# smritip/real-time-audio-sync

Measured on AMD Instinct MI355X. Metric: aligned chroma frames/sec, batch=64 OTW c=500; path-index match vs CPU ref, higher is better.
Workload: dtype f64 arithmetic, f32 features in HBM

## Files before the change

real_time_audio_sync_amd/csrc/otw.hip:

```cpp
#include <hip/hip_runtime.h>
#include <math.h>
#include <stddef.h>
#include <stdint.h>
#include <stdlib.h>
#include <string.h>
#include <type_traits>

#include "common.h"
#include "cost.h"

namespace rts {

constexpr int kF = 12;
constexpr int kFetch = 8;

struct OtwArgs {
    const void *ref;
    const void *live;
    const int32_t *live_len;
    int32_t *state;
    int32_t *path;
    double *bands;
    long long live_stride;
    int N, c, max_run_count, variant, cost_kind, mode;
// ... 89 lines not shown
__device__ __forceinline__ double wave_shift_up(double v, double lane0) {
    const int lo = __builtin_amdgcn_update_dpp(__double2loint(lane0), __double2loint(v), 0x138, 0xf, 0xf, false);
    const int hi = __builtin_amdgcn_update_dpp(__double2hiint(lane0), __double2hiint(v), 0x138, 0xf, 0xf, false);
    return __hiloint2double(hi, lo);
}

__device__ __forceinline__ double wave_bcast(double v, int src_lane) {
    const int lo = __builtin_amdgcn_readlane(__double2loint(v), src_lane);
    const int hi = __builtin_amdgcn_readlane(__double2hiint(v), src_lane);
    return __hiloint2double(hi, lo);
}

__device__ __forceinline__ double rfl(double v) {
    const int lo = __builtin_amdgcn_readfirstlane(__double2loint(v));
    const int hi = __builtin_amdgcn_readfirstlane(__double2hiint(v));
    return __hiloint2double(hi, lo);
}

#define RTS_DPP_MIN_STEP(CTRL, ROWMASK)                                                                       \
    do {                                                                                                      \
        const int tlo = __builtin_amdgcn_update_dpp(__double2loint(x), __double2loint(x), CTRL, ROWMASK, 0xf, false); \
        const int thi = __builtin_amdgcn_update_dpp(__double2hiint(x), __double2hiint(x), CTRL, ROWMASK, 0xf, false); \
        x = vmin(x, __hiloint2double(thi, tlo));                                                              \
    } while (0)

__device__ __forceinline__ double wave_min(double x) {
    RTS_DPP_MIN_STEP(0x111, 0xf);
    RTS_DPP_MIN_STEP(0x112, 0xf);
    RTS_DPP_MIN_STEP(0x114, 0xf);
    RTS_DPP_MIN_STEP(0x118, 0xf);
    RTS_DPP_MIN_STEP(0x142, 0xa);
    RTS_DPP_MIN_STEP(0x143, 0xc);
    return wave_bcast(x, 63);
}

__device__ __forceinline__ unsigned lds_addr(const double *p) {
    return (unsigned)(uintptr_t)(__attribute__((address_space(3))) const double *)p;
}
template <int OFF>
__device__ __forceinline__ double lds_read_imm(unsigned addr) {
    double r;
    asm volatile("ds_read_b64 %0, %1 offset:%2" : "=v"(r) : "v"(addr), "n"(OFF));
    return r;
}
template <int OFF>
__device__ __forceinline__ void lds_write_imm(unsigned addr, double v) {
    asm volatile("ds_write_b64 %0, %1 offset:%2" ::"v"(addr), "v"(v), "n"(OFF) : "memory");
}
template <int L, int R, int M = 0>
__device__ __forceinline__ void chain_load(unsigned bA, unsigned bB, unsigned dA, unsigned dB, double (&prevb)[L + 1],
                                           double (&D)[L]) {
    if constexpr (M <= L) {
        constexpr int off = ((R + M) & (L - 1)) * 65 * 8;
        constexpr bool wrap = (R + M) >= L;
        prevb[M] = lds_read_imm<off>(wrap ? bB : bA);
        if constexpr (M > 0) D[M - 1] = lds_read_imm<off>(wrap ? dB : dA);
        chain_load<L, R, M + 1>(bA, bB, dA, dB, prevb, D);
    }
}
template <int L, int M = 0>
__device__ __forceinline__ void chain_wait(double (&prevb)[L + 1], double (&D)[L]) {
    if constexpr (M == 0) asm volatile("s_waitcnt lgkmcnt(0)" ::: "memory");
    if constexpr (M <= L) {
        asm volatile("" : "+v"(prevb[M]));
        if constexpr (M < L) asm volatile("" : "+v"(D[M]));
        chain_wait<L, M + 1>(prevb, D);
// ... 748 lines not shown
template <int W, bool ALT>
__device__ __forceinline__ void otw_spec_strip(const double *Dv, const double *band, double *shadow, int pos, int c,
                                               int lane, double sentinel, OtwSpecOut *out, long long *rounds_acc = nullptr,
                                               bool prev0_sentinel = false) {
    const int k1 = (pos - c + 1 > 0) ? pos - c + 1 : 0;
    double fm;
    int fi;
    const double d_last = Dv[swz<W>(pos)];
    const double d_next = Dv[swz<W>(pos + 1)];
    int alt_ok = 0;
    strip_chain<W, false, true, ALT, true>(Dv, band, shadow, k1, pos - k1, (k1 > 0) ? sentinel : (double)INFINITY, lane, k1,
                                           fm, fi, nullptr, nullptr, 0, rounds_acc, prev0_sentinel, sentinel, &alt_ok);
    out->pmin[lane] = fm;
    out->pidx[lane] = fi;
    if (lane == 0) {
        out->k1 = k1;
        out->d = d_last;
        out->d2 = d_next;
        out->flag = alt_ok;
    }
}

template <int W>
__device__ __forceinline__ void otw_spec_argmin(double lm, int ml, int k1, double &g_out, int &idx_out) {
    constexpr int L = W / 64;
    const double g = wave_min(lm);
    const unsigned long long mask = __ballot(lm == g);
    const bool some = (g < INFINITY) && (mask != 0);
    const int first = (int)__builtin_ctzll(mask | (1ull << 63));
    g_out = g;
    idx_out = some ? k1 + L * first + __builtin_amdgcn_readlane(ml, first) : 0x7fffffff;
}

__device__ __forceinline__ double otw_last_cell_from(double prev_raw, int pos, int k1, double side_v, double diag_v, double d,
                                                     double sentinel) {
    const double inf = INFINITY;
    const int n = pos - k1;
    const double prev = (n > 0) ? prev_raw : ((k1 > 0) ? sentinel : inf);
    const double diag = (pos > 0) ? diag_v + 2 * d : inf;
    return vmin(vmin(side_v + d, diag), prev + d);
}
template <int W>
__device__ __forceinline__ double otw_last_cell(const double *band, int pos, int k1, double side_v, double diag_v, double d,
                                                double sentinel) {
    const int n = pos - k1;
    return otw_last_cell_from(band[swz<W>(pos - (n > 0 ? 1 : 0))], pos, k1, side_v, diag_v, d, sentinel);
}

template <int W, typename RT>
__device__ __forceinline__ OtwSettled otw_settle_hit_both(double *R, double *C, const OtwSpecOut *exr, const OtwSpecOut *exc,
                                                          OtwCtl &k, const OtwEnv &e, int pt, int j0, double sentinel) {
    const int c = e.c, lane = e.lane;
    const int jn = j0 + 1, t0 = pt - 1;
    if (e.deferred_update && k.pend_dir != -2) {
        k.run_count = (k.pend_dir == k.prev) ? k.run_count + 1 : 1;
        if (k.pend_dir != RTS_DIR_BOTH) k.prev = k.pend_dir;
        k.pend_dir = -2;
    }
    const int k1r_ = (j0 - c + 1 > 0) ? j0 - c + 1 : 0, k1c_ = (pt - c + 1 > 0) ? pt - c + 1 : 0;
    const double pra_raw = R[swz<W>(j0 - (j0 - k1r_ > 0 ? 1 : 0))], prb_raw = C[swz<W>(t0 - (t0 - k1c_ > 0 ? 1 : 0))];
    const double d1_raw = exr->d, d2_raw = exc->d, d3_raw = exc->d2, rlm = exr->pmin[lane], clm = exc->pmin[lane];
    const int rml = exr->pidx[lane], cml = exc->pidx[lane], rk1 = exr->k1, ck1 = exc->k1;
    const double d1 = rfl(d1_raw), d2 = rfl(d2_raw), d3 = rfl(d3_raw);
    double rmin, cmin;
    int ridx, cidx;
    otw_spec_argmin<W>(rlm, rml, __builtin_amdgcn_readfirstlane(rk1), rmin, ridx);
// ... 102 lines not shown
    k.cA = cl;
    k.cells += n + 1;
    OtwSettled o;
    o.row_fresh = is_row;
    o.col_fresh = !is_row;
    o.rf_min = o.cf_min = smin;
    o.rf_idx = o.cf_idx = sidx;
    o.row_corner = o.col_corner = true;
    o.rc = o.cc = cl;
    o.stop = false;
    return o;
}

#ifdef RTS_OTW_FULL_BARRIER
#define RTS_STEP_BARRIER() __syncthreads()
#else
#define RTS_STEP_BARRIER() ::rts::lds_barrier()
#endif

template <int W, int NW, bool DENSE, typename RT, bool SPEC>
__global__ void __launch_bounds__(64 * NW) __attribute__((amdgpu_waves_per_eu(kThroughput<RT> ? 6 : 1)))
otw_advance_kernel(OtwArgs a) {
    static_assert(!SPEC || (NW >= 8 && !DENSE), "the pipelined kernel needs 8 waves and no dense mirror");
    constexpr int NT = 64 * NW;
    constexpr int HW0 = SPEC ? 3 : (NW >= 4) ? 2 : 0;
    constexpr int NHELP = 64 * (NW - HW0);
#if defined(RTS_OTW_STAMPS) && RTS_OTW_STAMPS == 1
    long long stamp_sum[16] = {0, 0, 0, 0, 0, 0, 0, 0, 0, 0, 0, 0, 0, 0, 0, 0};
    int stamp_base = 0;
    long long stamp_last = (long long)__builtin_amdgcn_s_memtime();
    __builtin_amdgcn_s_waitcnt(0xC07F);
#endif
#if defined(RTS_OTW_STAMPS) && RTS_OTW_STAMPS == 2
    long long lw_hit = 0, lb_hit = 0, lw_oth = 0, lb_oth = 0, ln_hit = 0, ln_oth = 0, l_last = 0;
    long long lo_work = 0, lo_t0 = 0;
    long long lo_rounds = 0;
#define RTS_ROUNDS_ACC (&lo_rounds)
#define RTS_LW_BEGIN() do { lo_t0 = (long long)__builtin_amdgcn_s_memtime(); __builtin_amdgcn_s_waitcnt(0xC07F); } while (0)
#define RTS_LW_END(hit) do { const long long t_ = (long long)__builtin_amdgcn_s_memtime(); __builtin_amdgcn_s_waitcnt(0xC07F); if (hit) lo_work += t_ - lo_t0; } while (0)
#else
#define RTS_ROUNDS_ACC nullptr
#define RTS_LW_BEGIN() do { } while (0)
#define RTS_LW_END(hit) do { } while (0)
#endif
    extern __shared__ __align__(16) unsigned char smem_raw[];
    OtwLds<W, RT> &S = *reinterpret_cast<OtwLds<W, RT> *>(smem_raw);
    using LdsT = OtwLds<W, RT>;
    constexpr bool kNoLiveRing = !kHasLiveRing<RT>;
    constexpr bool kRefRing = !SPEC && !kNoLiveRing;
    constexpr size_t kSpecOff = (offsetof(LdsT, refw) + 15) & ~(size_t)15;
    OtwSpecLds<W> &SP = *reinterpret_cast<OtwSpecLds<W> *>(smem_raw + kSpecOff);

    const int tid = threadIdx.x;
    const int lane = tid & 63;
    const int wave = __builtin_amdgcn_readfirstlane(tid >> 6);
    const double sentinel = (a.variant == RTS_VARIANT_OTW) ? 1e10 : (double)INFINITY;
    const double inf = INFINITY;
    OtwEnv e;
    e.b = blockIdx.x;
    e.lane = lane;
    e.c = a.c;
    e.euclid = a.cost_kind == RTS_COST_EUCLID;
    e.variant = a.variant;
    e.mode = a.mode;
    e.max_run_count = a.max_run_count;
    e.path_cap = a.path_cap;
    e.live_f64 = a.live_f64;
    e.ref_f64 = a.ref_f64;
    e.live_base = (long long)e.b * a.live_stride * kF;
    e.live = a.live;
    if (a.ref_first) {
        const int nb = a.ref_len[e.b];
        e.N = nb;
        e.live_cap = 2 * nb;
        e.ref = static_cast<const char *>(a.ref) + a.ref_first[e.b] * (long long)kF * (a.ref_f64 ? 8 : 4);
    } else {
// ... 145 lines not shown
            S.j = k.j;
        }
    }
    __syncthreads();
    int buf = 0;
    OtwPlan pl;
    pl.t = pl.j0 = 0;
    pl.flags = kPlanExit;
    if constexpr (SPEC) {
        otw_costs_prime<W, RT>(S, e, S.t, S.j, tid, NT);
        if (wave == 0) {
            k.cA = rfl(S.R[swz<W>(k.j)]);
            k.cU = (k.t > 0) ? rfl(S.C[swz<W>(k.t - 1)]) : inf;
            k.cL = (k.j > 0) ? rfl(S.R[swz<W>(k.j - 1)]) : inf;
            pl = otw_make_plan<W, RT>(S, k, e, true);
        }
    } else {
        otw_precompute<W, RT>(S, e, S.t, S.j, S.Dr[0], S.Dc[0], tid, NT);
        if (wave == 0) otw_make_plan<W, RT>(S, k, e);
    }
    __syncthreads();

    int sp = 0;
#ifdef RTS_OTW_PRIO_W0
    if constexpr (SPEC) {
        if (wave == 0) __builtin_amdgcn_s_setprio(RTS_OTW_PRIO_W0);
        if (wave == 1 || wave == 2) __builtin_amdgcn_s_setprio(RTS_OTW_PRIO_W12);
    }
#endif
    if constexpr (SPEC) {
        if (wave >= HW0) {
            for (;;) {
                const int pt = __builtin_amdgcn_readfirstlane(S.plan_t[sp]), j0 = __builtin_amdgcn_readfirstlane(S.plan_j0[sp]);
                const int pflags = otw_resolve_plan(__builtin_amdgcn_readfirstlane(S.plan_flags[sp]), pt, c, &SP.col[sp]);
                if (pflags & kPlanExit) break;
                const bool do_row = (pflags & kPlanRow) != 0, do_col = (pflags & kPlanCol) != 0;
                RTS_LW_BEGIN();
                if constexpr (!kNoLiveRing)
                    if (wave == HW0) otw_refill<W, RT>(S, k, e, pt + 3, 0, false);
                if (!(pflags & kPlanHit)) RTS_STEP_BARRIER();
                if (!(pflags & kPlanStop))
                    otw_costs_advance<W, RT>(S, e, pt, j0 + (do_col ? 1 : 0), do_row, do_col, tid - 64 * HW0, NHELP);
                RTS_LW_END(pflags & kPlanHit);
                RTS_STEP_BARRIER();
                sp ^= 1;
            }
        } else if (wave == 1) {
            for (;;) {
                const int pt = __builtin_amdgcn_readfirstlane(S.plan_t[sp]), j0 = __builtin_amdgcn_readfirstlane(S.plan_j0[sp]);
                const int pflags = otw_resolve_plan(__builtin_amdgcn_readfirstlane(S.plan_flags[sp]), pt, c, &SP.col[sp]);
                if (pflags & kPlanExit) break;
                const int jn = j0 + ((pflags & kPlanCol) ? 1 : 0);
                double *R = (pflags & kPlanRi) ? SP.ShR : S.R, *Rsh = (pflags & kPlanRi) ? S.R : SP.ShR;
                RTS_LW_BEGIN();
                if (!(pflags & kPlanHit)) {
                    if ((pflags & (kPlanRow | kPlanCol | kPlanStop)) == (kPlanRow | kPlanCol))
                        otw_col_strip<W, DENSE, RT>(S, (pflags & kPlanCi) ? SP.ShC : S.C, a, e, S.Dc[(j0 + 1) & 1], pt,
                                                    j0 + 1, true, sentinel);
                    RTS_STEP_BARRIER();
                }
                if ((pflags & (kPlanHit | kPlanRow | kPlanCol)) == (kPlanHit | kPlanRow | kPlanCol)) {
                    const double av = otw_last_cell<W>(R, j0, (j0 - c + 1 > 0) ? j0 - c + 1 : 0, Rsh[swz<W>(j0)],
                                                       Rsh[swz<W>(j0 > 0 ? j0 - 1 : 0)], SP.row[sp].d, sentinel);
                    if (lane == 0) R[swz<W>(j0)] = av;
                }
                if (!(pflags & kPlanStop) && pt + 1 < live_len && pt + 1 < e.live_cap)
                    otw_spec_strip<W, false>(S.Dr[(pt + 1) & 1], R, Rsh, jn, c, lane, sentinel, &SP.row[sp ^ 1], RTS_ROUNDS_ACC);
                RTS_LW_END(pflags & kPlanHit);
                RTS_STEP_BARRIER();
                sp ^= 1;
            }
        } else if (wave == 2) {
            for (;;) {
                const int pt = __builtin_amdgcn_readfirstlane(S.plan_t[sp]), j0 = __builtin_amdgcn_readfirstlane(S.plan_j0[sp]);
                const int pflags = otw_resolve_plan(__builtin_amdgcn_readfirstlane(S.plan_flags[sp]), pt, c, &SP.col[sp]);
                if (pflags & kPlanExit) break;
                const int jn = j0 + ((pflags & kPlanCol) ? 1 : 0);
                double *C = (pflags & kPlanCi) ? SP.ShC : S.C, *Csh = (pflags & kPlanCi) ? S.C : SP.ShC;
                RTS_LW_BEGIN();
                if (!(pflags & kPlanHit)) {
                    if constexpr (kThroughput<RT>) {
                        const bool stop2 = (pflags & kPlanStop) != 0;
                        if (pflags & kPlanRow) {
                            double rf_min = inf;
                            int rf_idx = 0x7fffffff;
                            otw_row_strip<W, DENSE, RT>((pflags & kPlanRi) ? SP.ShR : S.R, a, e, S.Dr[pt & 1], pt, j0, jn, sentinel,
                                                        rf_min, rf_idx);
                            if (lane == 0) {
                                S.rfresh_min = rf_min;
                                S.rfresh_idx = rf_idx;
                            }
                        } else if ((pflags & kPlanCol) && !stop2) {
                            otw_col_strip<W, DENSE, RT>(S, C, a, e, S.Dc[jn & 1], pt, jn, false, sentinel);
                        }
                    }
                    RTS_STEP_BARRIER();
                }
                bool drop = false;
                if ((pflags & (kPlanHit | kPlanRow | kPlanCol)) == (kPlanHit | kPlanRow | kPlanCol)) {
                    const int t0 = pt - 1;
                    const double bv = otw_last_cell<W>(C, t0, (pt - c + 1 > 0) ? pt - c + 1 : 0, Csh[swz<W>(t0)],
                                                       Csh[swz<W>(t0 > 0 ? t0 - 1 : 0)], SP.col[sp].d, sentinel);
                    if (lane == 0) C[swz<W>(t0)] = bv;
                    drop = pt >= c;
                }
                if (!(pflags & kPlanStop) && jn + 1 < N)
                    otw_spec_strip<W, true>(S.Dc[(jn + 1) & 1], C, Csh, pt, c, lane, sentinel, &SP.col[sp ^ 1], RTS_ROUNDS_ACC, drop);
                RTS_LW_END(pflags & kPlanHit);
                RTS_STEP_BARRIER();
                sp ^= 1;
            }
        } else {
#if defined(RTS_OTW_STAMPS) && RTS_OTW_STAMPS == 2
            l_last = (long long)__builtin_amdgcn_s_memtime();
            __builtin_amdgcn_s_waitcnt(0xC07F);
#define RTS_W0_STEP_END(hit)                                              \
    do {                                                                  \
        const long long t0_ = (long long)__builtin_amdgcn_s_memtime();    \
        __builtin_amdgcn_s_waitcnt(0xC07F);                               \
        RTS_STEP_BARRIER();                                               \
        const long long t1_ = (long long)__builtin_amdgcn_s_memtime();    \
        __builtin_amdgcn_s_waitcnt(0xC07F);                               \
        if (hit) {                                                        \
            lw_hit += t0_ - l_last;                                       \
            lb_hit += t1_ - t0_;                                          \
            ln_hit += 1;                                                  \
        } else {                                                          \
            lw_oth += t0_ - l_last;                                       \
            lb_oth += t1_ - t0_;                                          \
            ln_oth += 1;                                                  \
        }                                                                 \
        l_last = t1_;                                                     \
    } while (0)
#else
#define RTS_W0_STEP_END(hit) RTS_STEP_BARRIER()
#endif
            int2 *const path_row = reinterpret_cast<int2 *>(e.path) + (size_t)e.b * e.path_cap;
            const auto hit_steps = [&](auto v2_c, auto defer_c) __attribute__((always_inline)) {
                constexpr bool V2 = decltype(v2_c)::value, DEFER = decltype(defer_c)::value;
#define RTS_RFL_CTL(f) k.f = __builtin_amdgcn_readfirstlane(k.f)
                RTS_RFL_CTL(t), RTS_RFL_CTL(j), RTS_RFL_CTL(dir), RTS_RFL_CTL(prev), RTS_RFL_CTL(run_count);
                RTS_RFL_CTL(status), RTS_RFL_CTL(n_path), RTS_RFL_CTL(consumed), RTS_RFL_CTL(rows), RTS_RFL_CTL(cols);
                RTS_RFL_CTL(truncated), RTS_RFL_CTL(pend_dir), RTS_RFL_CTL(pending_col), RTS_RFL_CTL(last_x);
                RTS_RFL_CTL(last_y), RTS_RFL_CTL(spec_valid), RTS_RFL_CTL(ri), RTS_RFL_CTL(ci);
#undef RTS_RFL_CTL
                for (;;) {
                    const int pt = __builtin_amdgcn_readfirstlane(pl.t), j0 = __builtin_amdgcn_readfirstlane(pl.j0);
                    const int fl = __builtin_amdgcn_readfirstlane(pl.flags);
                    const int kind = fl & (kPlanHit | kPlanRow | kPlanCol | kPlanStop | kPlanExit | kPlanHitIf);
                    const bool is_row = kind == (kPlanHit | kPlanRow);
                    if (!is_row && kind != (kPlanHit | kPlanCol)) return;
                    const int jn = is_row ? j0 : j0 + 1;
                    const int keep_lo = is_row ? pt - c + 1 : jn - c + 1;
                    const int keep_idx = __builtin_amdgcn_readfirstlane(is_row ? k.cb_idx : k.rb_idx);
                    if (keep_idx < ((keep_lo > 0) ? keep_lo : 0)) return;
#if defined(RTS_OTW_STAMPS) && RTS_OTW_STAMPS == 1
                    stamp_base = 0;
                    stamp_sum[6] += 1;
#endif
                    RTS_STAMP(0);
                    RTS_STAMP(1);
                    double *R = (fl & kPlanRi) ? SP.ShR : S.R, *C = (fl & kPlanCi) ? SP.ShC : S.C;
                    const int pos = is_row ? j0 : pt;
                    const int k1 = (pos - c + 1 > 0) ? pos - c + 1 : 0;
                    const int n = pos - k1;
                    double *band = is_row ? R : C, *other = is_row ? C : R;
                    const OtwSpecOut *ex = is_row ? &SP.row[sp] : &SP.col[sp];
                    if constexpr (DEFER) {
                        if (k.pend_dir != -2) {
                            k.run_count = (k.pend_dir == k.prev) ? k.run_count + 1 : 1;
                            if (k.pend_dir != RTS_DIR_BOTH) k.prev = k.pend_dir;
                            k.pend_dir = -2;
                        }
                    }
                    const double prev_raw = band[swz<W>(pos - (n > 0 ? 1 : 0))];
                    const double d = ex->d, lm = ex->pmin[lane];
                    const int ml = ex->pidx[lane], sk1 = ex->k1;
                    double smin;
                    int sidx;
                    otw_spec_argmin<W>(lm, ml, __builtin_amdgcn_readfirstlane(sk1), smin, sidx);
                    const double prev = (n > 0) ? prev_raw : ((k1 > 0) ? sentinel : inf);
                    const double diag = (pos > 0) ? (is_row ? k.cL : k.cU) + 2 * d : inf;
                    const double cl = vmin(vmin(k.cA + d, diag), prev + d);
                    if (lane == 0) {
                        band[swz<W>(pos)] = cl;
                        other[swz<W>(is_row ? pt : jn)] = cl;
                    }
                    if (is_row) {
                        k.rows += 1;
                        k.consumed = pt + 1;
                        k.cU = k.cA;
                        k.cL = prev;
                    } else {
                        k.cols += 1;
                        k.cL = k.cA;
                        k.cU = prev;
                    }
                    k.cA = cl;
                    k.cells += n + 1;
                    RTS_STAMP(3);
                    double rmin = is_row ? smin : k.rb_min, cmin = is_row ? k.cb_min : smin;
                    int ridx = is_row ? sidx : k.rb_idx, cidx = is_row ? k.cb_idx : sidx;
                    const bool r_new = cl < rmin, c_new = cl < cmin;
                    rmin = r_new ? cl : rmin;
                    ridx = r_new ? jn : ridx;
                    cmin = c_new ? cl : cmin;
                    cidx = c_new ? pt : cidx;
                    k.rb_min = rmin;
                    k.rb_idx = ridx;
                    k.cb_min = cmin;
                    k.cb_idx = cidx;
                    const bool rlt = rmin < cmin;
                    const int x = rlt ? pt : cidx, y = rlt ? ridx : jn;
                    bool append = true;
                    if constexpr (V2) {
                        const int xs = __builtin_amdgcn_readfirstlane(x), ys = __builtin_amdgcn_readfirstlane(y);
                        append = (k.n_path == 0) || (xs > k.last_x && ys >= k.last_y);
                        if (append) {
                            k.last_x = xs;
                            k.last_y = ys;
                        }
                    }
                    if (append) {
                        if (k.n_path < e.path_cap) {
                            if (lane == 0) path_row[k.n_path] = make_int2(x, y);
                        } else {
                            k.truncated = 1;
                        }
                        k.n_path += 1;
                    }
                    int nd = __builtin_amdgcn_readfirstlane((x < pt) ? RTS_DIR_COLUMN : (y < jn) ? RTS_DIR_ROW : RTS_DIR_BOTH);
                    if (pt < c)
                        nd = RTS_DIR_BOTH;
                    else if (k.run_count >= e.max_run_count)
                        nd = (k.prev == RTS_DIR_ROW) ? RTS_DIR_COLUMN : RTS_DIR_ROW;
                    if constexpr (DEFER) {
                        k.pend_dir = nd;
                    } else {
                        k.run_count = (nd == k.prev) ? k.run_count + 1 : 1;
                        if (nd != RTS_DIR_BOTH) k.prev = nd;
                    }
                    k.dir = nd;
                    k.pending_col = (nd == RTS_DIR_COLUMN);
                    k.t = pt;
                    k.j = jn;
                    RTS_STAMP(4);
                    k.spec_valid = 1;
                    pl = otw_make_plan<W, RT>(S, k, e, true, sp ^ 1);
                    RTS_STAMP(5);
                    RTS_W0_STEP_END(true);
                    sp ^= 1;
                }
            };
            for (;;) {
                if constexpr (W == 512 && !kThroughput<RT>) {
                    if (e.variant == RTS_VARIANT_LIVENOTE_V2) {
                        if (e.deferred_update)
                            hit_steps(std::true_type{}, std::true_type{});
                        else
                            hit_steps(std::true_type{}, std::false_type{});
                    } else if (e.deferred_update) {
                        hit_steps(std::false_type{}, std::true_type{});
                    } else {
                        hit_steps(std::false_type{}, std::false_type{});
                    }
                }
                RTS_STAMP2(0);
                const int pt = __builtin_amdgcn_readfirstlane(pl.t), j0 = __builtin_amdgcn_readfirstlane(pl.j0);
                pl.flags = __builtin_amdgcn_readfirstlane(pl.flags);
                const int pflags = otw_resolve_plan(pl.flags, pt, c, &SP.col[sp]);
                if (pflags & kPlanExit) break;
                if ((pl.flags & kPlanHitIf) && (pflags & kPlanHit)) {
                    k.ri ^= 1;
                    k.ci ^= 1;
                }
                const bool do_row = (pflags & kPlanRow) != 0, do_col = (pflags & kPlanCol) != 0;
                const bool stop = (pflags & kPlanStop) != 0;
                const int jn = j0 + (do_col ? 1 : 0);
                double *R = (pflags & kPlanRi) ? SP.ShR : S.R, *C = (pflags & kPlanCi) ? SP.ShC : S.C;
                OtwSettled o;
#if defined(RTS_OTW_STAMPS) && RTS_OTW_STAMPS == 1
                stamp_base = (pflags & kPlanHit) ? 0 : 8;
                if (stamp_base) stamp_sum[14] += 1; else stamp_sum[6] += 1;
#endif
                if (pflags & kPlanHit) RTS_STAMP(1);
                if ((pflags & kPlanHit) && do_row && do_col) {
                    o = otw_settle_hit_both<W, RT>(R, C, &SP.row[sp], &SP.col[sp], k, e, pt, j0, sentinel);
                } else if (pflags & kPlanHit) {
                    o = otw_settle_hit<W, RT>(R, C, do_row ? &SP.row[sp] : &SP.col[sp], k, e, pt, j0, do_row, sentinel);
                } else {
                    double rf_min = inf;
                    int rf_idx = 0x7fffffff;
                    if constexpr (!kThroughput<RT>) {
                        if (do_row)
                            otw_row_strip<W, DENSE, RT>(R, a, e, S.Dr[pt & 1], pt, j0, jn, sentinel, rf_min, rf_idx);
                        else if (do_col && !stop)
                            otw_col_strip<W, DENSE, RT>(S, C, a, e, S.Dc[jn & 1], pt, jn, false, sentinel);
                    }
                    RTS_STAMP(9);
                    RTS_STEP_BARRIER();
                    RTS_STAMP(10);
                    if constexpr (kThroughput<RT>) {
                        if (do_row) {
                            rf_min = rfl(S.rfresh_min);
                            rf_idx = __builtin_amdgcn_readfirstlane(S.rfresh_idx);
                        }
                    }
                    const double ld_u = C[swz<W>(pt > 0 ? pt - 1 : 0)], ld_l = R[swz<W>(jn > 0 ? jn - 1 : 0)];
                    o = otw_settle<W, DENSE, RT>(S, R, C, k, a, e, pt, j0, pflags, rf_min, rf_idx, sentinel);
                    k.cA = o.cc;
                    k.cU = (pt > 0) ? rfl(ld_u) : inf;
                    k.cL = (jn > 0) ? rfl(ld_l) : inf;
                }
                RTS_STAMP2(3);
                if (o.stop) {
                    k.status = RTS_STOP_REF_END;
                    k.t = pt;
                    k.j = jn;
                    k.pending_col = 0;
                } else {
                    otw_decide<W, RT>(R, C, k, e, pt, jn, o.row_fresh, o.rf_min, o.rf_idx, o.col_fresh, o.cf_min, o.cf_idx,
                                      o.row_corner, o.rc, o.col_corner, o.cc, false);
                }
                RTS_STAMP2(4);
                k.spec_valid = !o.stop;
                pl = otw_make_plan<W, RT>(S, k, e, true, sp ^ 1);
                RTS_STAMP2(5);
                RTS_W0_STEP_END(pflags & kPlanHit);
                sp ^= 1;
            }
#undef RTS_W0_STEP_END
        }
    } else if constexpr (NW >= 4) {
        if (wave >= HW0) {
            for (;;) {
                const int pt = __builtin_amdgcn_readfirstlane(S.plan_t[0]), j0 = __builtin_amdgcn_readfirstlane(S.plan_j0[0]),
                          pflags = __builtin_amdgcn_readfirstlane(S.plan_flags[0]);
                if (pflags & kPlanExit) break;
                const int jn = j0 + ((pflags & kPlanCol) ? 1 : 0);
                if (!(pflags & kPlanStop))
                    otw_precompute<W, RT>(S, e, pt, jn, S.Dr[buf ^ 1], S.Dc[buf ^ 1], tid - 64 * HW0, NHELP);
                __syncthreads();
                __syncthreads();
                buf ^= 1;
            }
        } else if (wave == 1) {
            for (;;) {
                const int pt = __builtin_amdgcn_readfirstlane(S.plan_t[0]), j0 = __builtin_amdgcn_readfirstlane(S.plan_j0[0]),
                          pflags = __builtin_amdgcn_readfirstlane(S.plan_flags[0]);
                if (pflags & kPlanExit) break;
                if ((pflags & (kPlanRow | kPlanCol | kPlanStop)) == (kPlanRow | kPlanCol))
                    otw_col_strip<W, DENSE, RT>(S, S.C, a, e, S.Dc[buf], pt, j0 + 1, true, sentinel);
                __syncthreads();
                __syncthreads();
                buf ^= 1;
            }
        } else {
            for (;;) {
                RTS_STAMP(0);
                const int pt = __builtin_amdgcn_readfirstlane(S.plan_t[0]), j0 = __builtin_amdgcn_readfirstlane(S.plan_j0[0]),
                          pflags = __builtin_amdgcn_readfirstlane(S.plan_flags[0]);
// ... 116 lines not shown
                }
                RTS_STAMP(7);
                otw_make_plan<W, RT>(S, k, e);
            }
            RTS_STAMP(8);
            __syncthreads();
            buf ^= 1;
        }
    }
    __syncthreads();

    {
        int te = S.t, je = S.j;
        const int t_state = te;
        if (te > e.live_cap - 1) te = e.live_cap - 1;
        if (je > N - 1) je = N - 1;
        double *bb = a.bands + (size_t)e.b * 2 * (c + 1);
        const double qnan = __longlong_as_double(0x7ff8000000000000LL);
        const int fl = S.plan_flags[sp];
        const double *Rf = (SPEC && (fl & kPlanRi)) ? SP.ShR : S.R, *Cf = (SPEC && (fl & kPlanCi)) ? SP.ShC : S.C;
        const bool row_missing = (t_state >= e.live_len) && (t_state <= e.live_cap - 1);
        const double sentinel = (e.variant == RTS_VARIANT_OTW) ? 1e10 : (double)INFINITY;
        for (int i = tid; i <= c; i += NT) {
            const int y = je - c + i, x = te - c + i;
            bb[i] = (y >= 0) ? (row_missing ? sentinel : Rf[swz<W>(y)]) : qnan;
            bb[(c + 1) + i] = (x >= 0 && x <= t_state) ? ((row_missing && x == t_state) ? sentinel : Cf[swz<W>(x)]) : qnan;
        }
    }
#if defined(RTS_OTW_STAMPS) && RTS_OTW_STAMPS == 1
    if (tid == 0 && a.debug)
        for (int i = 0; i < 16; i++) a.debug[(size_t)e.b * 16 + i] = stamp_sum[i];
#endif
#if defined(RTS_OTW_STAMPS) && RTS_OTW_STAMPS == 2
    if (tid == 0 && a.debug) {
        long long *dbg = a.debug + (size_t)e.b * 16;
        dbg[0] = lw_hit, dbg[1] = lb_hit, dbg[2] = ln_hit, dbg[3] = lw_oth, dbg[4] = lb_oth, dbg[5] = ln_oth;
    }
    if (a.debug && lane == 0 && wave >= 1 && wave <= 7) a.debug[(size_t)e.b * 16 + 5 + wave] = lo_work;
    if (a.debug && lane == 0 && wave >= 1 && wave <= 2) a.debug[(size_t)e.b * 16 + 12 + wave] = lo_rounds;
#endif
    if (tid == 0) {
        st[RTS_ST_T] = k.t;
        st[RTS_ST_J] = k.j;
        st[RTS_ST_DIRECTION] = e.deferred_update ? RTS_DIR_BOTH : k.dir;
        st[RTS_ST_PREVIOUS] = k.prev;
        st[RTS_ST_RUN_COUNT] = k.run_count;
        st[RTS_ST_STATUS] = k.status;
        st[RTS_ST_FIRST_INSERT] = k.first;
        st[RTS_ST_N_PATH] = k.n_path;
        st[RTS_ST_CONSUMED] = k.consumed;
        st[RTS_ST_ROW_STRIPS] = k.rows;
        st[RTS_ST_COL_STRIPS] = k.cols;
        st[RTS_ST_CELLS_LO] = (int32_t)(uint32_t)(k.cells & 0xffffffffLL);
        st[RTS_ST_CELLS_HI] = (int32_t)(uint32_t)((unsigned long long)k.cells >> 32);
        st[RTS_ST_PATH_TRUNCATED] = k.truncated;
        st[14] = k.pend_dir;
        st[RTS_ST_BAND_RECOMPUTES] = k.recomputes;
    }
}

__device__ __forceinline__ void otw_fresh_state(int32_t *st, int variant) {
    for (int i = 0; i < RTS_STATE_LEN; i++) st[i] = 0;
    st[RTS_ST_DIRECTION] = RTS_DIR_BOTH;
    st[RTS_ST_PREVIOUS] = RTS_DIR_NONE;
    st[RTS_ST_RUN_COUNT] = (variant == RTS_VARIANT_OTW) ? 1 : 0;
    st[RTS_ST_STATUS] = RTS_RUNNING;
    st[RTS_ST_FIRST_INSERT] = 1;
    st[14] = -2;
}

__global__ void otw_reset_kernel(int32_t *state, int B, int variant) {
    const int b = blockIdx.x * blockDim.x + threadIdx.x;
// ... 650 lines not shown
    hipStream_t s = (hipStream_t)stream;
    RTS_HIP(hipMemcpyAsync(state, h->state + (size_t)b * RTS_STATE_LEN, sizeof(int32_t) * RTS_STATE_LEN,
                           hipMemcpyDeviceToHost, s));
    RTS_HIP(hipStreamSynchronize(s));
    state[14] = 0;
    return RTS_OK;
}

int rts_otw_read_path(rts_otw *h, int b, int32_t *pairs, int cap_pairs, int *n, void *stream) {
    using namespace rts;
    if (!h || !n) return set_error(RTS_ERR_INVALID, "NULL argument");
    return read_path(h->state, RTS_STATE_LEN, RTS_ST_N_PATH, h->path, h->path_cap, b, h->B, pairs, cap_pairs, n,
                     (hipStream_t)stream);
}

int rts_otw_read_bands(rts_otw *h, int b, double *row_band, double *col_band, void *stream) {
    using namespace rts;
    if (!h || !row_band || !col_band) return set_error(RTS_ERR_INVALID, "NULL argument");
    if (b < 0 || b >= h->B) return set_error(RTS_ERR_INVALID, "stream index %d out of range [0, %d)", b, h->B);
    hipStream_t s = (hipStream_t)stream;
    const double *bb = h->bands + (size_t)b * 2 * (h->c + 1);
    RTS_HIP(hipMemcpyAsync(row_band, bb, sizeof(double) * (h->c + 1), hipMemcpyDeviceToHost, s));
    RTS_HIP(hipMemcpyAsync(col_band, bb + (h->c + 1), sizeof(double) * (h->c + 1), hipMemcpyDeviceToHost, s));
    RTS_HIP(hipStreamSynchronize(s));
    return RTS_OK;
}

#ifdef RTS_OTW_STAMPS
int rts_otw_set_debug(rts_otw *h, long long *debug_dev) {
    if (!h) return rts::set_error(RTS_ERR_INVALID, "handle is NULL");
    h->debug = debug_dev;
    return RTS_OK;
}
#endif

int rts_otw_device_views(rts_otw *h, int32_t **path_dev, int *path_cap, int32_t **state_dev) {
    using namespace rts;
    if (!h) return set_error(RTS_ERR_INVALID, "handle is NULL");
    if (path_dev) *path_dev = h->path;
    if (path_cap) *path_cap = h->path_cap;
    if (state_dev) *state_dev = h->state;
    return RTS_OK;
}

}
```

Before: 33.27 million.

## Handle speculative both-direction steps in wave-0 hit loop with paired argmin

Extends wave 0's fast speculative hit loop so that steps advancing both row and column, including the hit-if case, are settled inline instead of falling back to the slower general path. A new paired wave-min reduction interleaves the DPP steps for the row and column argmins to overlap their latencies. It also reworks the debug timestamp instrumentation into per-step-kind buckets. The cost is more branching and register pressure in the hot wave-0 loop, and new correctness-sensitive band bookkeeping.

Result: faster. 34.12 million, median of 6 (+2.5%).

```diff
diff --git a/real_time_audio_sync_amd/csrc/otw.hip b/real_time_audio_sync_amd/csrc/otw.hip
--- a/real_time_audio_sync_amd/csrc/otw.hip
+++ b/real_time_audio_sync_amd/csrc/otw.hip
@@ -145,6 +145,29 @@
     RTS_DPP_MIN_STEP(0x142, 0xa);
     RTS_DPP_MIN_STEP(0x143, 0xc);
     return wave_bcast(x, 63);
+}
+
+__device__ __forceinline__ void wave_min2(double &x0, double &x1) {
+#define RTS_DPP_MIN_STEP2(CTRL, ROWMASK) \
+    do {                                 \
+        {                                \
+            double &x = x0;              \
+            RTS_DPP_MIN_STEP(CTRL, ROWMASK); \
+        }                                \
+        {                                \
+            double &x = x1;              \
+            RTS_DPP_MIN_STEP(CTRL, ROWMASK); \
+        }                                \
+    } while (0)
+    RTS_DPP_MIN_STEP2(0x111, 0xf);
+    RTS_DPP_MIN_STEP2(0x112, 0xf);
+    RTS_DPP_MIN_STEP2(0x114, 0xf);
+    RTS_DPP_MIN_STEP2(0x118, 0xf);
+    RTS_DPP_MIN_STEP2(0x142, 0xa);
+    RTS_DPP_MIN_STEP2(0x143, 0xc);
+#undef RTS_DPP_MIN_STEP2
+    x0 = wave_bcast(x0, 63);
+    x1 = wave_bcast(x1, 63);
 }
 
 __device__ __forceinline__ unsigned lds_addr(const double *p) {
@@ -959,6 +982,21 @@
     idx_out = some ? k1 + L * first + __builtin_amdgcn_readlane(ml, first) : 0x7fffffff;
 }
 
+template <int W>
+__device__ __forceinline__ void otw_spec_argmin2(double rlm, int rml, int rk1, double clm, int cml, int ck1, double &rg_out,
+                                                 int &ridx_out, double &cg_out, int &cidx_out) {
+    constexpr int L = W / 64;
+    double rg = rlm, cg = clm;
+    wave_min2(rg, cg);
+    const unsigned long long rmask = __ballot(rlm == rg), cmask = __ballot(clm == cg);
+    const bool rsome = (rg < INFINITY) && (rmask != 0), csome = (cg < INFINITY) && (cmask != 0);
+    const int rfirst = (int)__builtin_ctzll(rmask | (1ull << 63)), cfirst = (int)__builtin_ctzll(cmask | (1ull << 63));
+    rg_out = rg;
+    cg_out = cg;
+    ridx_out = rsome ? rk1 + L * rfirst + __builtin_amdgcn_readlane(rml, rfirst) : 0x7fffffff;
+    cidx_out = csome ? ck1 + L * cfirst + __builtin_amdgcn_readlane(cml, cfirst) : 0x7fffffff;
+}
+
 __device__ __forceinline__ double otw_last_cell_from(double prev_raw, int pos, int k1, double side_v, double diag_v, double d,
                                                      double sentinel) {
     const double inf = INFINITY;
@@ -1127,16 +1165,30 @@
     __builtin_amdgcn_s_waitcnt(0xC07F);
 #endif
 #if defined(RTS_OTW_STAMPS) && RTS_OTW_STAMPS == 2
-    long long lw_hit = 0, lb_hit = 0, lw_oth = 0, lb_oth = 0, ln_hit = 0, ln_oth = 0, l_last = 0;
-    long long lo_work = 0, lo_t0 = 0;
+    long long lw_k0 = 0, lw_k1 = 0, lw_k2 = 0, lw_k3 = 0;
+    long long lb_k0 = 0, lb_k1 = 0, lb_k2 = 0, lb_k3 = 0;
+    long long ln_k0 = 0, ln_k1 = 0, ln_k2 = 0, ln_k3 = 0;
+    long long l_last = 0;
+    long long lo_k0 = 0, lo_k1 = 0, lo_k2 = 0, lo_t0 = 0;
     long long lo_rounds = 0;
 #define RTS_ROUNDS_ACC (&lo_rounds)
+#define RTS_STEP_KIND(raw, res)                                                                          \
+    (!((res) & kPlanHit) ? 3 : (((res) & (kPlanRow | kPlanCol)) != (kPlanRow | kPlanCol)) ? 0 : ((raw) & kPlanHitIf) ? 2 : 1)
 #define RTS_LW_BEGIN() do { lo_t0 = (long long)__builtin_amdgcn_s_memtime(); __builtin_amdgcn_s_waitcnt(0xC07F); } while (0)
-#define RTS_LW_END(hit) do { const long long t_ = (long long)__builtin_amdgcn_s_memtime(); __builtin_amdgcn_s_waitcnt(0xC07F); if (hit) lo_work += t_ - lo_t0; } while (0)
+#define RTS_LW_END(kind)                                                  \
+    do {                                                                  \
+        const long long t_ = (long long)__builtin_amdgcn_s_memtime();     \
+        __builtin_amdgcn_s_waitcnt(0xC07F);                               \
+        const int kd_ = (kind);                                           \
+        if (kd_ == 0) lo_k0 += t_ - lo_t0;                                \
+        if (kd_ == 1) lo_k1 += t_ - lo_t0;                                \
+        if (kd_ == 2) lo_k2 += t_ - lo_t0;                                \
+    } while (0)
 #else
 #define RTS_ROUNDS_ACC nullptr
+#define RTS_STEP_KIND(raw, res) 0
 #define RTS_LW_BEGIN() do { } while (0)
-#define RTS_LW_END(hit) do { } while (0)
+#define RTS_LW_END(kind) do { } while (0)
 #endif
     extern __shared__ __align__(16) unsigned char smem_raw[];
     OtwLds<W, RT> &S = *reinterpret_cast<OtwLds<W, RT> *>(smem_raw);
@@ -1348,7 +1400,8 @@
         if (wave >= HW0) {
             for (;;) {
                 const int pt = __builtin_amdgcn_readfirstlane(S.plan_t[sp]), j0 = __builtin_amdgcn_readfirstlane(S.plan_j0[sp]);
-                const int pflags = otw_resolve_plan(__builtin_amdgcn_readfirstlane(S.plan_flags[sp]), pt, c, &SP.col[sp]);
+                const int praw = __builtin_amdgcn_readfirstlane(S.plan_flags[sp]);
+                const int pflags = otw_resolve_plan(praw, pt, c, &SP.col[sp]);
                 if (pflags & kPlanExit) break;
                 const bool do_row = (pflags & kPlanRow) != 0, do_col = (pflags & kPlanCol) != 0;
                 RTS_LW_BEGIN();
@@ -1357,14 +1410,15 @@
                 if (!(pflags & kPlanHit)) RTS_STEP_BARRIER();
                 if (!(pflags & kPlanStop))
                     otw_costs_advance<W, RT>(S, e, pt, j0 + (do_col ? 1 : 0), do_row, do_col, tid - 64 * HW0, NHELP);
-                RTS_LW_END(pflags & kPlanHit);
+                RTS_LW_END(RTS_STEP_KIND(praw, pflags));
                 RTS_STEP_BARRIER();
                 sp ^= 1;
             }
         } else if (wave == 1) {
             for (;;) {
                 const int pt = __builtin_amdgcn_readfirstlane(S.plan_t[sp]), j0 = __builtin_amdgcn_readfirstlane(S.plan_j0[sp]);
-                const int pflags = otw_resolve_plan(__builtin_amdgcn_readfirstlane(S.plan_flags[sp]), pt, c, &SP.col[sp]);
+                const int praw = __builtin_amdgcn_readfirstlane(S.plan_flags[sp]);
+                const int pflags = otw_resolve_plan(praw, pt, c, &SP.col[sp]);
                 if (pflags & kPlanExit) break;
                 const int jn = j0 + ((pflags & kPlanCol) ? 1 : 0);
                 double *R = (pflags & kPlanRi) ? SP.ShR : S.R, *Rsh = (pflags & kPlanRi) ? S.R : SP.ShR;
@@ -1382,14 +1436,15 @@
                 }
                 if (!(pflags & kPlanStop) && pt + 1 < live_len && pt + 1 < e.live_cap)
                     otw_spec_strip<W, false>(S.Dr[(pt + 1) & 1], R, Rsh, jn, c, lane, sentinel, &SP.row[sp ^ 1], RTS_ROUNDS_ACC);
-                RTS_LW_END(pflags & kPlanHit);
+                RTS_LW_END(RTS_STEP_KIND(praw, pflags));
                 RTS_STEP_BARRIER();
                 sp ^= 1;
             }
         } else if (wave == 2) {
             for (;;) {
                 const int pt = __builtin_amdgcn_readfirstlane(S.plan_t[sp]), j0 = __builtin_amdgcn_readfirstlane(S.plan_j0[sp]);
-                const int pflags = otw_resolve_plan(__builtin_amdgcn_readfirstlane(S.plan_flags[sp]), pt, c, &SP.col[sp]);
+                const int praw = __builtin_amdgcn_readfirstlane(S.plan_flags[sp]);
+                const int pflags = otw_resolve_plan(praw, pt, c, &SP.col[sp]);
                 if (pflags & kPlanExit) break;
                 const int jn = j0 + ((pflags & kPlanCol) ? 1 : 0);
                 double *C = (pflags & kPlanCi) ? SP.ShC : S.C, *Csh = (pflags & kPlanCi) ? S.C : SP.ShC;
@@ -1422,7 +1477,7 @@
                 }
                 if (!(pflags & kPlanStop) && jn + 1 < N)
                     otw_spec_strip<W, true>(S.Dc[(jn + 1) & 1], C, Csh, pt, c, lane, sentinel, &SP.col[sp ^ 1], RTS_ROUNDS_ACC, drop);
-                RTS_LW_END(pflags & kPlanHit);
+                RTS_LW_END(RTS_STEP_KIND(praw, pflags));
                 RTS_STEP_BARRIER();
                 sp ^= 1;
             }
@@ -1430,30 +1485,31 @@
 #if defined(RTS_OTW_STAMPS) && RTS_OTW_STAMPS == 2
             l_last = (long long)__builtin_amdgcn_s_memtime();
             __builtin_amdgcn_s_waitcnt(0xC07F);
-#define RTS_W0_STEP_END(hit)                                              \
+#define RTS_W0_STEP_END(kind)                                             \
     do {                                                                  \
         const long long t0_ = (long long)__builtin_amdgcn_s_memtime();    \
         __builtin_amdgcn_s_waitcnt(0xC07F);                               \
         RTS_STEP_BARRIER();                                               \
         const long long t1_ = (long long)__builtin_amdgcn_s_memtime();    \
         __builtin_amdgcn_s_waitcnt(0xC07F);                               \
-        if (hit) {                                                        \
-            lw_hit += t0_ - l_last;                                       \
-            lb_hit += t1_ - t0_;                                          \
-            ln_hit += 1;                                                  \
-        } else {                                                          \
-            lw_oth += t0_ - l_last;                                       \
-            lb_oth += t1_ - t0_;                                          \
-            ln_oth += 1;                                                  \
-        }                                                                 \
+        const int kd_ = (kind);                                           \
+        if (kd_ == 0) lw_k0 += t0_ - l_last, lb_k0 += t1_ - t0_, ln_k0 += 1; \
+        if (kd_ == 1) lw_k1 += t0_ - l_last, lb_k1 += t1_ - t0_, ln_k1 += 1; \
+        if (kd_ == 2) lw_k2 += t0_ - l_last, lb_k2 += t1_ - t0_, ln_k2 += 1; \
+        if (kd_ == 3) lw_k3 += t0_ - l_last, lb_k3 += t1_ - t0_, ln_k3 += 1; \
         l_last = t1_;                                                     \
     } while (0)
 #else
-#define RTS_W0_STEP_END(hit) RTS_STEP_BARRIER()
+#define RTS_W0_STEP_END(kind) RTS_STEP_BARRIER()
 #endif
             int2 *const path_row = reinterpret_cast<int2 *>(e.path) + (size_t)e.b * e.path_cap;
             const auto hit_steps = [&](auto v2_c, auto defer_c) __attribute__((always_inline)) {
                 constexpr bool V2 = decltype(v2_c)::value, DEFER = decltype(defer_c)::value;
+#ifdef RTS_OTW_NO_BOTH_LOOP
+                constexpr bool kBothHere = false;
+#else
+                constexpr bool kBothHere = true;
+#endif
 #define RTS_RFL_CTL(f) k.f = __builtin_amdgcn_readfirstlane(k.f)
                 RTS_RFL_CTL(t), RTS_RFL_CTL(j), RTS_RFL_CTL(dir), RTS_RFL_CTL(prev), RTS_RFL_CTL(run_count);
                 RTS_RFL_CTL(status), RTS_RFL_CTL(n_path), RTS_RFL_CTL(consumed), RTS_RFL_CTL(rows), RTS_RFL_CTL(cols);
@@ -1465,58 +1521,128 @@
                     const int fl = __builtin_amdgcn_readfirstlane(pl.flags);
                     const int kind = fl & (kPlanHit | kPlanRow | kPlanCol | kPlanStop | kPlanExit | kPlanHitIf);
                     const bool is_row = kind == (kPlanHit | kPlanRow);
-                    if (!is_row && kind != (kPlanHit | kPlanCol)) return;
+                    const bool hit_if = kind == (kPlanHitIf | kPlanRow | kPlanCol);
+                    const bool is_both = kBothHere && (hit_if || kind == (kPlanHit | kPlanRow | kPlanCol));
+                    if (!is_row && !is_both && kind != (kPlanHit | kPlanCol)) return;
                     const int jn = is_row ? j0 : j0 + 1;
-                    const int keep_lo = is_row ? pt - c + 1 : jn - c + 1;
-                    const int keep_idx = __builtin_amdgcn_readfirstlane(is_row ? k.cb_idx : k.rb_idx);
-                    if (keep_idx < ((keep_lo > 0) ? keep_lo : 0)) return;
+                    double rmin, cmin, cl;
+                    int ridx, cidx;
+                    if (is_both) {
 #if defined(RTS_OTW_STAMPS) && RTS_OTW_STAMPS == 1
-                    stamp_base = 0;
-                    stamp_sum[6] += 1;
+                        stamp_base = 0;
 #endif
-                    RTS_STAMP(0);
-                    RTS_STAMP(1);
-                    double *R = (fl & kPlanRi) ? SP.ShR : S.R, *C = (fl & kPlanCi) ? SP.ShC : S.C;
-                    const int pos = is_row ? j0 : pt;
-                    const int k1 = (pos - c + 1 > 0) ? pos - c + 1 : 0;
-                    const int n = pos - k1;
-                    double *band = is_row ? R : C, *other = is_row ? C : R;
-                    const OtwSpecOut *ex = is_row ? &SP.row[sp] : &SP.col[sp];
-                    if constexpr (DEFER) {
-                        if (k.pend_dir != -2) {
-                            k.run_count = (k.pend_dir == k.prev) ? k.run_count + 1 : 1;
-                            if (k.pend_dir != RTS_DIR_BOTH) k.prev = k.pend_dir;
-                            k.pend_dir = -2;
+                        RTS_STAMP(0);
+                        RTS_STAMP(1);
+                        const int flr = hit_if ? ((fl | kPlanHit) ^ (kPlanRi | kPlanCi)) : fl;
+                        double *R = (flr & kPlanRi) ? SP.ShR : S.R, *C = (flr & kPlanCi) ? SP.ShC : S.C;
+                        const int t0 = pt - 1;
+                        const int k1r = (j0 - c + 1 > 0) ? j0 - c + 1 : 0, k1c = (pt - c + 1 > 0) ? pt - c + 1 : 0;
+                        const int lo_r = (jn - c + 1 > 0) ? jn - c + 1 : 0;
+                        const int k1c_s = (t0 - c + 1 > 0) ? t0 - c + 1 : 0;
+                        const OtwSpecOut *exr = &SP.row[sp], *exc = &SP.col[sp];
+                        const double pra = R[swz<W>(j0 - (j0 - k1r > 0 ? 1 : 0))], prb = C[swz<W>(t0 - (t0 - k1c > 0 ? 1 : 0))];
+                        const double d1_raw = exr->d, d2_raw = exc->d, d3_raw = exc->d2, rlm = exr->pmin[lane], clm = exc->pmin[lane];
+                        const int rml = exr->pidx[lane], cml = exc->pidx[lane];
+                        const int cflag = exc->flag;
+                        if (hit_if && !(pt < c || __builtin_amdgcn_readfirstlane(cflag) != 0)) return;
+                        const double d1 = rfl(d1_raw), d2 = rfl(d2_raw), d3 = rfl(d3_raw);
+                        const double av = otw_last_cell_from(rfl(pra), j0, k1r, k.cA, k.cL, d1, sentinel);
+                        const double bv = otw_last_cell_from(rfl(prb), t0, k1c, k.cA, k.cU, d2, sentinel);
+                        const double cl_both = vmin(vmin(av + d3, k.cA + 2 * d3), bv + d3);
+                        double rsm, csm;
+                        int rsi, csi;
+                        otw_spec_argmin2<W>(rlm, rml, k1r, clm, cml, k1c_s, rsm, rsi, csm, csi);
+                        const bool a_new = av < rsm, b_new = bv < csm;
+                        rmin = a_new ? av : rsm;
+                        cmin = b_new ? bv : csm;
+                        ridx = __builtin_amdgcn_readfirstlane(a_new ? j0 : rsi);
+                        cidx = __builtin_amdgcn_readfirstlane(b_new ? t0 : csi);
+                        if (ridx < lo_r || cidx < k1c) return;
+#if defined(RTS_OTW_STAMPS) && RTS_OTW_STAMPS == 1
+                        stamp_sum[6] += 1;
+#endif
+                        if constexpr (DEFER) {
+                            if (k.pend_dir != -2) {
+                                k.run_count = (k.pend_dir == k.prev) ? k.run_count + 1 : 1;
+                                if (k.pend_dir != RTS_DIR_BOTH) k.prev = k.pend_dir;
+                                k.pend_dir = -2;
+                            }
                         }
+                        cl = cl_both;
+                        if (lane == 0) {
+                            R[swz<W>(j0)] = av;
+                            C[swz<W>(t0)] = bv;
+                            R[swz<W>(jn)] = cl;
+                            C[swz<W>(pt)] = cl;
+                            if (k1c > k1c_s) {
+                                double sv = sentinel;
+                                asm volatile("" : "+v"(sv));
+                                C[swz<W>(k1c - 1)] = sv;
+                            }
+                        }
+                        k.rows += 1;
+                        k.cols += 1;
+                        k.consumed = pt + 1;
+                        k.cells += (j0 - k1r + 1) + (pt - k1c + 1);
+                        k.cU = bv;
+                        k.cL = av;
+                        k.cA = cl;
+                        RTS_STAMP(3);
+                    } else {
+                        const int keep_lo = is_row ? pt - c + 1 : jn - c + 1;
+                        const int keep_idx = __builtin_amdgcn_readfirstlane(is_row ? k.cb_idx : k.rb_idx);
+                        if (keep_idx < ((keep_lo > 0) ? keep_lo : 0)) return;
+#if defined(RTS_OTW_STAMPS) && RTS_OTW_STAMPS == 1
+                        stamp_base = 0;
+                        stamp_sum[6] += 1;
+#endif
+                        RTS_STAMP(0);
+                        RTS_STAMP(1);
+                        double *R = (fl & kPlanRi) ? SP.ShR : S.R, *C = (fl & kPlanCi) ? SP.ShC : S.C;
+                        const int pos = is_row ? j0 : pt;
+                        const int k1 = (pos - c + 1 > 0) ? pos - c + 1 : 0;
+                        const int n = pos - k1;
+                        double *band = is_row ? R : C, *other = is_row ? C : R;
+                        const OtwSpecOut *ex = is_row ? &SP.row[sp] : &SP.col[sp];
+                        if constexpr (DEFER) {
+                            if (k.pend_dir != -2) {
+                                k.run_count = (k.pend_dir == k.prev) ? k.run_count + 1 : 1;
+                                if (k.pend_dir != RTS_DIR_BOTH) k.prev = k.pend_dir;
+                                k.pend_dir = -2;
+                            }
+                        }
+                        const double prev_raw = band[swz<W>(pos - (n > 0 ? 1 : 0))];
+                        const double d = ex->d, lm = ex->pmin[lane];
+                        const int ml = ex->pidx[lane], sk1 = ex->k1;
+                        double smin;
+                        int sidx;
+                        otw_spec_argmin<W>(lm, ml, __builtin_amdgcn_readfirstlane(sk1), smin, sidx);
+                        const double prev = (n > 0) ? prev_raw : ((k1 > 0) ? sentinel : inf);
+                        const double diag = (pos > 0) ? (is_row ? k.cL : k.cU) + 2 * d : inf;
+                        cl = vmin(vmin(k.cA + d, diag), prev + d);
+                        if (lane == 0) {
+                            band[swz<W>(pos)] = cl;
+                            other[swz<W>(is_row ? pt : jn)] = cl;
+                        }
+                        if (is_row) {
+                            k.rows += 1;
+                            k.consumed = pt + 1;
+                            k.cU = k.cA;
+                            k.cL = prev;
+                        } else {
+                            k.cols += 1;
+                            k.cL = k.cA;
+                            k.cU = prev;
+                        }
+                        k.cA = cl;
+                        k.cells += n + 1;
+                        RTS_STAMP(3);
+                        rmin = is_row ? smin : k.rb_min, cmin = is_row ? k.cb_min : smin;
+                        ridx = is_row ? sidx : k.rb_idx, cidx = is_row ? k.cb_idx : sidx;
                     }
-                    const double prev_raw = band[swz<W>(pos - (n > 0 ? 1 : 0))];
-                    const double d = ex->d, lm = ex->pmin[lane];
-                    const int ml = ex->pidx[lane], sk1 = ex->k1;
-                    double smin;
-                    int sidx;
-                    otw_spec_argmin<W>(lm, ml, __builtin_amdgcn_readfirstlane(sk1), smin, sidx);
-                    const double prev = (n > 0) ? prev_raw : ((k1 > 0) ? sentinel : inf);
-                    const double diag = (pos > 0) ? (is_row ? k.cL : k.cU) + 2 * d : inf;
-                    const double cl = vmin(vmin(k.cA + d, diag), prev + d);
-                    if (lane == 0) {
-                        band[swz<W>(pos)] = cl;
-                        other[swz<W>(is_row ? pt : jn)] = cl;
-                    }
-                    if (is_row) {
-                        k.rows += 1;
-                        k.consumed = pt + 1;
-                        k.cU = k.cA;
-                        k.cL = prev;
-                    } else {
-                        k.cols += 1;
-                        k.cL = k.cA;
-                        k.cU = prev;
-                    }
-                    k.cA = cl;
-                    k.cells += n + 1;
-                    RTS_STAMP(3);
-                    double rmin = is_row ? smin : k.rb_min, cmin = is_row ? k.cb_min : smin;
-                    int ridx = is_row ? sidx : k.rb_idx, cidx = is_row ? k.cb_idx : sidx;
+                    const int flip = (is_both && hit_if) ? 1 : 0;
+                    k.ri ^= flip;
+                    k.ci ^= flip;
                     const bool r_new = cl < rmin, c_new = cl < cmin;
                     rmin = r_new ? cl : rmin;
                     ridx = r_new ? jn : ridx;
@@ -1564,7 +1690,7 @@
                     k.spec_valid = 1;
                     pl = otw_make_plan<W, RT>(S, k, e, true, sp ^ 1);
                     RTS_STAMP(5);
-                    RTS_W0_STEP_END(true);
+                    RTS_W0_STEP_END(is_both ? (hit_if ? 2 : 1) : 0);
                     sp ^= 1;
                 }
             };
@@ -1584,9 +1710,10 @@
                 RTS_STAMP2(0);
                 const int pt = __builtin_amdgcn_readfirstlane(pl.t), j0 = __builtin_amdgcn_readfirstlane(pl.j0);
                 pl.flags = __builtin_amdgcn_readfirstlane(pl.flags);
-                const int pflags = otw_resolve_plan(pl.flags, pt, c, &SP.col[sp]);
+                const int praw = pl.flags;
+                const int pflags = otw_resolve_plan(praw, pt, c, &SP.col[sp]);
                 if (pflags & kPlanExit) break;
-                if ((pl.flags & kPlanHitIf) && (pflags & kPlanHit)) {
+                if ((praw & kPlanHitIf) && (pflags & kPlanHit)) {
                     k.ri ^= 1;
                     k.ci ^= 1;
                 }
@@ -1642,7 +1769,7 @@
                 k.spec_valid = !o.stop;
                 pl = otw_make_plan<W, RT>(S, k, e, true, sp ^ 1);
                 RTS_STAMP2(5);
-                RTS_W0_STEP_END(pflags & kPlanHit);
+                RTS_W0_STEP_END(RTS_STEP_KIND(praw, pflags));
                 sp ^= 1;
             }
 #undef RTS_W0_STEP_END
@@ -1825,12 +1952,15 @@
         for (int i = 0; i < 16; i++) a.debug[(size_t)e.b * 16 + i] = stamp_sum[i];
 #endif
 #if defined(RTS_OTW_STAMPS) && RTS_OTW_STAMPS == 2
-    if (tid == 0 && a.debug) {
-        long long *dbg = a.debug + (size_t)e.b * 16;
-        dbg[0] = lw_hit, dbg[1] = lb_hit, dbg[2] = ln_hit, dbg[3] = lw_oth, dbg[4] = lb_oth, dbg[5] = ln_oth;
-    }
-    if (a.debug && lane == 0 && wave >= 1 && wave <= 7) a.debug[(size_t)e.b * 16 + 5 + wave] = lo_work;
-    if (a.debug && lane == 0 && wave >= 1 && wave <= 2) a.debug[(size_t)e.b * 16 + 12 + wave] = lo_rounds;
+    if (a.debug) {
+        long long *dbg = a.debug + (size_t)e.b * 64;
+        if (tid == 0) {
+            dbg[0] = lw_k0, dbg[1] = lb_k0, dbg[2] = ln_k0, dbg[16] = lw_k1, dbg[17] = lb_k1, dbg[18] = ln_k1;
+            dbg[32] = lw_k2, dbg[33] = lb_k2, dbg[34] = ln_k2, dbg[48] = lw_k3, dbg[49] = lb_k3, dbg[50] = ln_k3;
+        }
+        if (lane == 0 && wave >= 1 && wave <= 7) dbg[2 + wave] = lo_k0, dbg[18 + wave] = lo_k1, dbg[34 + wave] = lo_k2;
+        if (lane == 0 && wave >= 1 && wave <= 2) dbg[9 + wave] = lo_rounds;
+    }
 #endif
     if (tid == 0) {
         st[RTS_ST_T] = k.t;
@@ -2547,6 +2677,8 @@
     h->debug = debug_dev;
     return RTS_OK;
 }
+int rts_otw_stamp_level(void) { return RTS_OTW_STAMPS; }
+int rts_otw_debug_words(void) { return (RTS_OTW_STAMPS == 2) ? 64 : 16; }
 #endif
 
 int rts_otw_device_views(rts_otw *h, int32_t **path_dev, int *path_cap, int32_t **state_dev) {
```
